# illini-robomaster/irmv_detection

Hardware: AMD Instinct MI355X
Metric: end-to-end FPS (preprocess→NMS→PnP) 640×640 YOLOv8n, 1/2/4/8 MI355X (higher is better)
Workload: dtype f16

## Files before the change

### irmv_detection_amd/csrc/engine.cpp

```cpp
#include "engine_internal.hpp"

static thread_local std::string g_err;
int irmv::fail(int code, const std::string &msg) { g_err = msg; return code; }

extern "C" const char *irmv_last_error(void) { return g_err.c_str(); }
extern "C" const char *irmv_version(void)
{
    static char buf[96];
    static std::once_flag once;
    std::call_once(once, [] {
        int v = 0;
        if (hipRuntimeGetVersion(&v) != hipSuccess) v = 0;
        snprintf(buf, sizeof buf, "irmv_hip 0.3 (gfx950; HIP runtime %d)", v);
    });
    return buf;
}
extern "C" int irmv_device_synchronize(int device)
{
    HIP_TRY(hipSetDevice(device));
    HIP_TRY(hipDeviceSynchronize());
    return IRMV_OK;
}
extern "C" int irmv_device_count(int *count)
{
// ... 188 lines not shown
    cfg->armor_min_large_center_distance = 3.2; cfg->armor_max_large_center_distance = 5.5;
    cfg->src_format = IRMV_SRC_HWC8;
    cfg->bayer_gain_q8[0] = cfg->bayer_gain_q8[1] = cfg->bayer_gain_q8[2] = 256;
}

static EngineSwitches read_switches()
{
    auto set = [](const char *name) { return getenv(name) != nullptr; };
    auto starts = [](const char *name, char c) { const char *v = getenv(name); return v && v[0] == c; };
    auto off = [&](const char *name) { return starts(name, '0'); };
    auto is1 = [&](const char *name) { return starts(name, '1'); };
    EngineSwitches s;
    TuneSwitches &t = s.tune;
    t.untuned = off("IRMV_AUTOTUNE"); t.verbose = set("IRMV_AUTOTUNE_VERBOSE"); t.warn = set("IRMV_TUNE_WARN");
    const char *s2 = getenv("IRMV_FORCE_S2"), *wres = getenv("IRMV_FORCE_WRES");
    t.has_s2 = s2 != nullptr; t.force_s2 = s2 ? s2 : "";
    t.has_wres = wres != nullptr; t.force_wres = wres ? wres : "";
    t.force_pw = set("IRMV_FORCE_PW"); t.force_pwn = set("IRMV_FORCE_PWN"); t.force_cm = set("IRMV_FORCE_CM");
    t.force_w8 = set("IRMV_FORCE_W8"); t.force_nt8 = set("IRMV_FORCE_NT8"); t.force_pf4 = set("IRMV_FORCE_PF4");
    t.no_pw = set("IRMV_NO_PW"); t.no_pwn = set("IRMV_NO_PWN"); t.no_pf2 = set("IRMV_NO_PF2"); t.no_pf4 = set("IRMV_NO_PF4");
    t.no_cm = set("IRMV_NO_CM"); t.no_w8 = set("IRMV_NO_W8"); t.no_nt8 = set("IRMV_NO_NT8"); t.no_wres = set("IRMV_NO_WRES");
    t.no_deep = is1("IRMV_NO_DEEP");
    s.front.fastx = !off("IRMV_FRONT_FASTX"); s.front.direct = !off("IRMV_FRONT_DIRECT"); s.front.tall = !off("IRMV_FRONT_TILE8");
    s.fused_front = !off("IRMV_FUSED_FRONT"); s.fused_c2f = !off("IRMV_FUSED_C2F"); s.bneck64 = !off("IRMV_BNECK64"); s.kpt3 = !off("IRMV_KPT3");
    s.fused_head = !off("IRMV_FUSED_HEAD");
    s.merge_head0 = off("IRMV_MERGE_HEAD0") ? 0 : (is1("IRMV_MERGE_HEAD0") ? 1 : -1);
    s.group_head = !off("IRMV_GROUP_HEAD"); s.group_verbose = set("IRMV_GROUP_VERBOSE"); s.group_force = set("IRMV_GROUP_FORCE");
    if (const char *ns = getenv("IRMV_STREAMS")) { s.has_streams = true; s.streams = atoi(ns); }
    s.numa = !off("IRMV_NUMA");
    s.inline_copies = is1("IRMV_INLINE_COPIES"); s.graph_upload = !off("IRMV_GRAPH_UPLOAD"); s.window_upload = !off("IRMV_WINDOW_UPLOAD");
    if (const char *uk = getenv("IRMV_UPLOAD_KERNEL")) s.upload_kernel_blocks = atoi(uk);
    s.sync_launch = starts("IRMV_SYNC_LAUNCH", 'e') ? 1 : (starts("IRMV_SYNC_LAUNCH", 'g') ? 0 : -1);
    s.split_scan = !off("IRMV_SPLIT_SCAN"); s.emit_scan = !off("IRMV_EMIT_SCAN");
    s.sparse_head = !off("IRMV_SPARSE_HEAD"); s.sparse_branch = !off("IRMV_SPARSE_BRANCH");
    s.zero_copy_results = !off("IRMV_ZERO_COPY_RESULTS"); s.post_keys_only = is1("IRMV_POST_KEYS_ONLY");
    s.nms_classwalk = !off("IRMV_NMS_CLASSWALK");
    s.nms_prefilter = off("IRMV_NMS_PREFILTER") ? 0 : 1;
    if (const char *pe = getenv("IRMV_NMS_PRE")) { int hi = 0, lo = 0; if (sscanf(pe, "%d,%d", &hi, &lo) == 2 && hi >= 64 && hi <= 512 && lo >= 32 && lo < hi) s.nms_prefilter = hi | (lo << 16); }
    if (const char *st = getenv("IRMV_NMS_STAMPS")) { s.nms_stamps = true; s.nms_stamps_slots = atoi(st); }
    return s;
}

constexpr size_t kCfgSizeV1 = offsetof(irmv_engine_cfg, src_format);
constexpr size_t kCfgSizeV2 = offsetof(irmv_engine_cfg, reserved2);
static_assert(offsetof(irmv_engine_cfg, net_height) < kCfgSizeV2 && kCfgSizeV2 < sizeof(irmv_engine_cfg), "three distinct cfg sizes");
static_assert(offsetof(irmv_engine_cfg, win_width) == offsetof(irmv_engine_cfg, reserved2) + 4 && offsetof(irmv_engine_cfg, win_height) + 2 == sizeof(irmv_engine_cfg),
              "win_width / win_height fill the tail of irmv_engine_cfg");

static irmv_engine_cfg window_view(const irmv_engine_cfg &c)
{
    irmv_engine_cfg v = c;
    if (c.win_width > 0 && c.win_height > 0) { v.src_width = c.win_width; v.src_height = c.win_height; }
    v.win_width = v.win_height = 0;
    return v;
}

static int resolve_cfg(const irmv_engine_cfg *cfg_in, irmv_engine_cfg *full)
{
    const size_t sz = cfg_in->struct_size;
    if (sz != sizeof(irmv_engine_cfg) && sz != kCfgSizeV1 && sz != kCfgSizeV2) return fail(IRMV_ERR_ARG, "irmv_engine_cfg size mismatch");
    if (sz != sizeof(irmv_engine_cfg)) {
        irmv_engine_cfg_default(full);
        memcpy(full, cfg_in, sz == kCfgSizeV1 ? kCfgSizeV1 : offsetof(irmv_engine_cfg, net_height));
        full->struct_size = sizeof *full;
        full->bayer_demosaic = IRMV_DEMOSAIC_BILINEAR;
    } else {
        *full = *cfg_in;
// ... 339 lines not shown
```

### irmv_detection_amd/csrc/engine_internal.hpp

```cpp
#pragma once
#include <hip/hip_runtime.h>

#include <algorithm>
#include <chrono>
#include <cmath>
#include <cstdio>
#include <cstring>
#include <fstream>
#include <map>
#include <mutex>
#include <set>
#include <memory>
#include <string>
#include <vector>

#include "../../include/irmv_hip.h"
#include "irmv_common.hpp"
#include "numa.hpp"

using namespace irmv;

namespace irmv { int fail(int code, const std::string &msg); }
#define HIP_TRY(expr)                                                                                 \
    do {                                                                                              \
// ... 27 lines not shown
};

struct SegRef { int t = -1, coff = 0, C = 0, shift = 0; };

struct FrontSwitches { bool fastx = true, direct = true, tall = true; };

struct TuneSwitches {
    bool untuned, verbose, warn;
    bool has_s2, has_wres;
    std::string force_s2, force_wres;
    bool force_pw, force_pwn, force_cm, force_w8, force_nt8, force_pf4;
    bool no_pw, no_pwn, no_pf2, no_pf4, no_cm, no_w8, no_nt8, no_wres, no_deep;
};

struct EngineSwitches {
    TuneSwitches tune{};
    FrontSwitches front;
    bool fused_front = true, fused_c2f = true;
    bool bneck64 = true;
    bool kpt3 = true;
    bool fused_head = true;
    int merge_head0 = -1;
    bool group_head = true;
    bool group_verbose = false;
    bool group_force = false;
    bool has_streams = false; int streams = 0;
    bool numa = true;
    bool inline_copies = false;
    bool graph_upload = true;
    int upload_kernel_blocks = 256;
    bool window_upload = true;
    int sync_launch = -1;
    bool split_scan = true;
    bool emit_scan = true, sparse_head = true, sparse_branch = true;
    bool zero_copy_results = true;
    bool post_keys_only = false;
    bool nms_classwalk = true;
    int nms_prefilter = 1;
    bool nms_stamps = false; int nms_stamps_slots = 0;
};

enum OpKind { OP_PRE, OP_CONV0, OP_CONV, OP_POOL, OP_NMS, OP_LIGHT, OP_FRONT, OP_C2F2, OP_C2F32, OP_DW, OP_SHUF, OP_SCAN, OP_BNECK, OP_KPT3, OP_DEMOSAIC, OP_CROP };

struct Op {
    OpKind kind;
    std::string layer;
    ConvCfg cfg{};
    ConvCfg cfg_one{};
    char kname_one[48] = {0};
    SegRef s0, s1;
    int Hin = 0, Win = 0, Hout = 0, Wout = 0, cin = 0, cout = 0, cout_pad = 0, ksteps = 0;
    int out_t = -1, out_coff = 0, res_t = -1, res_coff = 0;
    half_t *w_packed = nullptr;
    half_t *w_k16 = nullptr;
    half_t *w_lds[4] = {nullptr, nullptr, nullptr, nullptr};
    float *bias = nullptr;
    double flops = 0, bytes = 0;
    double w_bytes = 0;
    double out_bytes = 0;
    bool pair = false;
    int level = -1;
    char kname[48] = {0};
    int sub[4] = {-1, -1, -1, -1};
    int mode = 0;
    bool shortcut = false;
    int fuse_next = -1;
// ... 167 lines not shown
```

### irmv_detection_amd/csrc/engine_plan.cpp

```cpp
#include "engine_internal.hpp"

static bool is_cls_final_carrier(const Op &op) { return op.fuse_next >= 0 && op.level >= 0 && op.layer.rfind("model.22.cv3.", 0) == 0; }

void irmv::finalize_head_fusion(irmv_engine *e)
{
    for (Op &op : e->ops) {
        if (op.fuse_next < 0) continue;
        const bool k16 = op.cfg.cin16 && !op.cfg.lds && !op.cfg_one.lds && !op.cfg.deep && !op.cfg_one.deep && op.cfg.nt == 1 && op.cfg_one.nt == 1 && e->ops[op.fuse_next].w_k16;
        const bool ok = k16 || (op.cfg.lds && op.cfg.nt == 4 && op.cfg_one.lds && op.cfg_one.nt == 4);
        if (!ok) { op.fuse_next = -1; continue; }
        e->ops[op.fuse_next].fused_away = true;
        e->lazy_tensors.insert(e->tensors[op.out_t].name);
        const size_t l = strlen(op.kname), l1 = strlen(op.kname_one);
        snprintf(op.kname + l, sizeof op.kname - l, "+1x1");
        snprintf(op.kname_one + l1, sizeof op.kname_one - l1, "+1x1");
    }
    int fused = 0;
    for (const Op &op : e->ops) fused += is_cls_final_carrier(op);
    e->emit_scan = e->sw.split_scan && fused == 3 && e->sw.emit_scan;
    e->sparse_head = e->emit_scan && e->cand_bits && e->sw.sparse_head;
    e->sparse_branch = e->sparse_head && e->sw.sparse_branch;
}

static bool is_box_final_carrier(const Op &op) { return op.fuse_next >= 0 && op.level >= 0 && op.layer.rfind("model.22.cv2.", 0) == 0; }

static void sparse_head_plan(irmv_engine *e, std::vector<Launch> &plan)
{
    int last_cls = -1;
    bool lvl_cls[3] = {false, false, false};
    for (size_t i = 0; i < plan.size(); i++)
        if (plan[i].scan && plan[i].group < 0) { last_cls = (int)i; lvl_cls[e->ops[plan[i].op].level] = true; }
    auto box_carrier = [&](const Launch &l) {
        const Op &op = e->ops[l.op];
        return l.group < 0 && l.fused && op.kind == OP_CONV && is_box_final_carrier(op) && op.level < 3 && lvl_cls[op.level];
    };
    std::vector<char> first_conv(plan.size(), 0);
    if (e->sparse_branch)
        for (size_t i = 0; i < plan.size(); i++) {
            const Launch &f = plan[i];
            const Op &fo = e->ops[f.op];
            if (f.group >= 0 || f.fused || f.scan || fo.kind != OP_CONV || !(f.cfg_one ? fo.cfg_one : fo.cfg).wr || fo.res_t >= 0) continue;
            int carrier = -1;
            for (size_t j = i + 1; j < plan.size(); j++) {
                const Op &co = e->ops[plan[j].op];
                if (box_carrier(plan[j]) && co.level == fo.level && co.s0.t == fo.out_t && co.s1.C == 0 && co.s0.coff == fo.out_coff && co.Hin == fo.Hout && co.Win == fo.Wout) carrier = plan[j].op;
            }
            bool other = false;
            for (int k = 0; k < (int)e->ops.size(); k++) {
                const Op &o = e->ops[k];
                if (k == carrier || k == f.op) continue;
                other = other || o.s0.t == fo.out_t || o.s1.t == fo.out_t || o.res_t == fo.out_t || o.out_t == fo.out_t;
            }
            first_conv[i] = carrier >= 0 && !other;
        }
    std::vector<Launch> out, moved;
    for (size_t i = 0; i < plan.size(); i++) {
        Launch &l = plan[i];
        Op &op = e->ops[l.op];
        if (l.scan) {
            if (l.group < 0) l.bytes -= e->ops[op.fuse_next].out_bytes;
            else for (size_t m = 0; m < e->head_groups[l.group].members.size(); m++)
                if (l.scan >> m & 1u) l.bytes -= e->ops[e->ops[e->head_groups[l.group].members[m]].fuse_next].out_bytes;
        }
        const bool cls_first = op.level >= 0 && op.level < 3 && lvl_cls[op.level];
        const bool box = box_carrier(l);
        const bool kpt = op.kind == OP_KPT3 && cls_first && (int)i > last_cls;
        if (box || kpt) {
            l.sparse = true;
            l.bytes -= box ? e->ops[op.fuse_next].out_bytes : op.out_bytes;
            if (e->sparse_branch) l.gate = 1;
        }
        if (first_conv[i]) {
            l.gate = 2;
            op.gated_first = true;
// ... 54 lines not shown
```

### irmv_detection_amd/csrc/irmv_common.hpp

```cpp
#pragma once

#include <hip/hip_runtime.h>

#include <cstdint>
#include <cstdlib>

namespace irmv {

typedef _Float16 half_t;
typedef _Float16 half8 __attribute__((ext_vector_type(8)));
typedef _Float16 half4 __attribute__((ext_vector_type(4)));
typedef float f32x4 __attribute__((ext_vector_type(4)));

constexpr float kActScale = 1.44269504088896341f;
constexpr float kActUnscale = 0.693147180559945309f;
typedef unsigned int u32x4_t __attribute__((ext_vector_type(4)));
__device__ __forceinline__ float silu_rcp(float y) { return __builtin_amdgcn_rcpf(1.0f + __builtin_amdgcn_exp2f(-y)); }
__device__ __forceinline__ unsigned int silu_pack2(float y0, float y1)
{
    const float r0 = silu_rcp(y0), r1 = silu_rcp(y1);
    unsigned int o;
    asm("v_fma_mixlo_f16 %0, %1, %2, 0" : "=v"(o) : "v"(y0), "v"(r0));
    asm("v_fma_mixhi_f16 %0, %1, %2, 0" : "+v"(o) : "v"(y1), "v"(r1));
    return o;
// ... 245 lines not shown
    const half_t *wl;
    int tiles_x, tiles_y, twc_log2, patch_bytes, batch, tile2d;
    int gx, gy;
};
struct LdsMultiArgs {
    int n;
    int start[kMultiMax + 1];
    LdsMember m[kMultiMax];
};
struct DirectMultiArgs {
    int n;
    int start[kMultiMax + 1], gx[kMultiMax], gy[kMultiMax];
    ConvArgs a[kMultiMax];
};

struct ConvCfg {
    int ks, stride, mt, nt; bool cin16; int act; bool out_f32; bool lds; int ipw;
    bool deep;
    bool ct;
    bool pw;
    bool pf2;
    bool pf4;
    bool w8;
    int cm;
    bool wr;
    bool pp;
};
struct ConvWeights { const half_t *w_packed; const half_t *w_lds[4]; const half_t *w_k16; };
struct ConvLaunch;
bool resolve_conv(const ConvCfg &cfg, const ConvArgs &a, const ConvWeights &w, int batch, ConvLaunch *out = nullptr);
bool launch_conv(const ConvCfg &cfg, const ConvArgs &a, const ConvWeights &w, int batch, hipStream_t s);
const char *conv_cfg_name(const ConvCfg &cfg, char *buf, int n);
bool conv_pw_eligible(const ConvCfg &cfg, const ConvArgs &a);
bool conv_lds_fits(const ConvArgs &a, const ConvWeights &w, int stride, int mt, int nt);
int conv_wres_tiles(const ConvArgs &a, int stride, bool pp);
bool launch_conv_lds_multi(int nt, const ConvArgs *a, const ConvWeights *w, int n, int batch, hipStream_t s);
bool launch_conv_direct_multi(const ConvCfg &cfg, const ConvArgs *a, int n, hipStream_t s);

void launch_sppf_pool(half_t *buf, int batch, int H, int W, int C, hipStream_t s);
int sppf_slab(int batch, int H, int W, int C);

struct DevDet {
    float box_net[4];
    float xyxy[4];
    float score;
    int32_t cls, anchor, pnp_ok;
    float kpts_net[8];
    float kpts[8];
    double rvec[3], tvec[3], quat[4];
    int32_t armor_valid;
    int32_t armor_size;
    int32_t n_lights;
    int32_t pad_;
};
struct DevFrameOut { int32_t num_dets, n_candidates, overflow, pad; };

struct PnpConst {
    double fx, fy, cx, cy, k1, k2, p1, p2, k3;
    double hy[2], hz[2];
};

struct PostArgs {
    const float *head_all;
    int slots_total, first;
    float *boxes;
    unsigned long long *keys;
// ... 78 lines not shown
```

### irmv_detection_amd/csrc/k_conv.hip

```cpp
#include "irmv_common.hpp"

#include <algorithm>
#include <cstdio>
#include <cstring>
#include <iterator>
#include <mutex>
#include <type_traits>

namespace irmv {

template <int MT, int NT>
struct PrefetchDepth { static constexpr int value = (MT * NT >= 8) ? 2 : ((MT * NT >= 4) ? 3 : 4); };
template <int MT, int NT>
struct DeepPrefetchDepth { static constexpr int value = (MT + NT <= 2) ? 12 : ((MT + NT <= 3) ? 10 : 6); };


template <int KS, int STRIDE, int MT, int NT, bool CIN16, int ACT, bool OUT_F32, bool CT = false, bool DEEP = false>
__device__ __forceinline__ void conv_mfma_body(const ConvArgs &a, int wg_x, int wg_y, int grid_x, int grid_y)
{
    constexpr int PAD = KS / 2;
    constexpr int PF = DEEP ? DeepPrefetchDepth<MT, NT>::value : PrefetchDepth<MT, NT>::value;
    static_assert(!CT || (KS == 3 && !CIN16), "chunk-major order is the 3x3 LDS family's");
    const int lane = threadIdx.x & 63, wave = threadIdx.x >> 6;
    const int g = lane >> 4, r = lane & 15;
// ... 605 lines not shown
    const int units = (a.M + 15) / 16;
    int wg = (cus[dev] * per_cu[dev] + groups - 1) / groups;
    if (wg > (units + 7) / 8) wg = (units + 7) / 8;
    if (wg < 1) wg = 1;
    hipLaunchKernelGGL((conv1x1_pwn_kernel<KS, NBW>), dim3(wg, groups), dim3(512), lds, s, a, wg);
}

static constexpr struct { int ksteps, nbw; ConvLauncher launch; } k_pw[] = {
    {4, 1, launch_pw_inst<4>}, {6, 1, launch_pw_inst<6>}, {8, 1, launch_pw_inst<8>}, {12, 1, launch_pw_inst<12>}, {16, 1, launch_pw_inst<16>},
    {4, 2, launch_pwn_inst<4, 2>}, {6, 2, launch_pwn_inst<6, 2>}, {8, 2, launch_pwn_inst<8, 2>}, {12, 2, launch_pwn_inst<12, 2>}, {16, 2, launch_pwn_inst<16, 2>},
    {4, 4, launch_pwn_inst<4, 4>}, {6, 4, launch_pwn_inst<6, 4>}, {8, 4, launch_pwn_inst<8, 4>},
};

static ConvLauncher pick_pw(const ConvCfg &c, const ConvArgs &a, LdsGeom &g)
{
    const int nbw = c.ipw > 1 ? c.ipw : 1;
    if (!conv_pw_eligible(c, a) || a.cout_pad % (64 * nbw) != 0) return nullptr;
    for (const auto &v : k_pw)
        if (v.ksteps == a.ksteps && v.nbw == nbw) {
            g.bytes = (size_t)nbw * 4 * a.ksteps * 1024 + (nbw > 1 ? (size_t)nbw * 64 * 4 : 0);
            return v.launch;
        }
    return nullptr;
}

constexpr int lds_pmax(int stride, int mt, bool tile2d, int wr = 0, int pf = 0)
{
    return pf == 2 ? (stride == 1 ? 4 : 8) : (wr ? 4 : ((tile2d && stride == 1) ? (mt == 4 ? 8 : 4) : 12));
}

#ifndef IRMV_LDS_WAVES
#define IRMV_LDS_WAVES 2
#endif
template <int STRIDE, int MT, int NT, bool TILE2D, int N2, int PF = 0, int CM = 0, int NWV = 4, int WR = 0, bool PP = false>
__device__ __forceinline__ void conv3x3_lds_body(const ConvArgs &a, const half_t *wl, int tiles_x, int tiles_y, int twc_log2, int a_patch_bytes, int ipw, int batch,
                                                 int wg_x, int wg_y, int grid_x, int grid_y, int stagger = 0)
{
    extern __shared__ __attribute__((aligned(16))) unsigned char smem[];
    const int lane = threadIdx.x & 63, wave = threadIdx.x >> 6, tid = threadIdx.x;
    constexpr bool PF2 = PF != 0;
    constexpr int NPF = PF == 2 ? 4 : (PF == 1 ? 2 : 1);
    constexpr int NTH = 64 * NWV;
    static_assert(!PP || (WR > 0 && NWV % 2 == 0), "ping-pong groups share resident weights");
    constexpr int NWP = PP ? NWV / 2 : NWV;
    constexpr int NTP = 64 * NWP;
    const int sub = PP ? wave / NWP : 0, wv = wave - sub * NWP, tidp = tid - sub * NTP;
    const int g = lane >> 4, r = lane & 15;
    const int bx = wg_x, by = wg_y;
    (void)grid_x; (void)grid_y;
    const int wg_tiles = PP ? (tiles_x * tiles_y + 1) / 2 : tiles_x * tiles_y;
    const int grp = bx / wg_tiles;
    int tile = PP ? 2 * (bx - grp * wg_tiles) + sub : bx - grp * wg_tiles;
    const bool active = tile < tiles_x * tiles_y;
    if (!active) tile = 0;
    const int img = grp * ipw, nimg = min(ipw, batch - img);
    const int nblk = by;
    const int HWo = a.Hout * a.Wout;
    bool gated = false;
    unsigned int l_mask = 0u;
    int l_pos = 0;
    int n_mine = nimg, n_max = nimg;
    if constexpr (WR > 0) {
        auto gate_images = [&](int t) -> unsigned int {
            const int h = a.tile_gate - 1;
            int nseg, lo0, len, pitch;
            if constexpr (TILE2D) {
                const int TWc = 1 << twc_log2, RH = NWP * MT * (16 >> twc_log2);
                const int tyi = t / tiles_x, txi = t - tyi * tiles_x;
                const int ya = max(tyi * RH - h, 0), yb = min(tyi * RH + RH + h, a.Hout);
                const int xa = max(txi * TWc - h, 0), xb = min(txi * TWc + TWc + h, a.Wout);
                nseg = yb - ya; lo0 = ya * a.Wout + xa; len = xb - xa; pitch = a.Wout;
            } else {
                constexpr int TPX = 16 * NWP * MT;
                const int lo = max(t * TPX - h * (a.Wout + 1), 0), hi = min(min(t * TPX + TPX, HWo) + h * (a.Wout + 1), HWo);
                nseg = 1; lo0 = lo; len = hi - lo; pitch = 0;
            }
            const int wps = (len + 62) >> 5, items = nseg * wps;
            unsigned int m = 0u;
            for (int j0 = 0; j0 < items; j0 += 64) {
                const int it = j0 + lane, sg = it / wps, bl = a.scan_abase + lo0 + sg * pitch, wd = (bl >> 5) + (it - sg * wps);
                const int s0 = max(bl - wd * 32, 0), s1 = min(bl + len - wd * 32, 32);
                const bool item = it < items && s1 > s0;
                const unsigned int bm = item ? (0xffffffffu >> (32 - (s1 - s0))) << s0 : 0u;
                for (int i0 = 0; i0 < nimg; i0 += 16) {
                    unsigned int cw[16];
#pragma unroll
                    for (int i = 0; i < 16; i++) cw[i] = i0 + i < nimg ? a.cand_bits[(unsigned int)((img + i0 + i) * a.cand_words + (item ? wd : 0))] : 0u;
#pragma unroll
                    for (int i = 0; i < 16; i++) m |= __ballot((cw[i] & bm) != 0u) != 0ull ? 1u << ((i0 + i) & 31) : 0u;
                }
            }
            return (unsigned int)__builtin_amdgcn_readfirstlane((int)m);
        };
        gated = a.tile_gate != 0 && a.cand_bits != nullptr && nimg <= 32;
        if (gated) {
// ... 64 lines not shown
    constexpr int PMAX = lds_pmax(STRIDE, MT, TILE2D, WR, PF);
    constexpr int WPT = (9 * NT * 64 + NTH - 1) / NTH;
    const int n_pe = PR * PW * 4;
    const float inv_pw = 1.0f / (float)PW;
    const half_t *src_p[PMAX];
    int dst_p[PMAX];
    bool val_p[PMAX], use_p[PMAX];
#pragma unroll
    for (int i = 0; i < PMAX; i++) {
        const int e = tidp + i * NTP;
        use_p[i] = e < n_pe;
        val_p[i] = false;
        src_p[i] = a.s0.p;
        dst_p[i] = 0;
        if (i * NTP >= n_pe) continue;
        const int pix = use_p[i] ? (e >> 2) : 0, q = e & 3;
        int pr = (int)((float)pix * inv_pw);
        pr -= (pr * PW > pix) ? 1 : 0;
        pr += ((pr + 1) * PW <= pix) ? 1 : 0;
        const int pc = pix - pr * PW;
        const int iy = iy_base + pr, ix = ix_base + pc;
        val_p[i] = active && use_p[i] && (unsigned)iy < (unsigned)a.Hin && (unsigned)ix < (unsigned)a.Win;
        src_p[i] = a.s0.p + ((size_t)(img * a.Hin + (val_p[i] ? iy : 0)) * a.Win + (val_p[i] ? ix : 0)) * a.s0.ld + q * 8;
        dst_p[i] = pix * pix_stride(STRIDE) + q * 16;
    }
    const half8 *wsrc = reinterpret_cast<const half8 *>(wl) + (size_t)nblk * chunks * (9 * NT * 64);

    const half8 *w2 = s_w2 + lane;

    half8 rp[NPF][PMAX], rw[NPF][WPT];
    const size_t img_stride = (size_t)a.Hin * a.Win * a.s0.ld;
    int l_im = 0, l_chunk = 0;
    int c_im = 0, c_chunk = 0;
    auto issue_loads = [&](half8 (&p)[PMAX], half8 (&w)[WPT]) {
        const size_t off = (size_t)l_im * img_stride + (size_t)l_chunk * 32;
#pragma unroll
        for (int i = 0; i < PMAX; i++) {
            p[i] = zero8;
            if (val_p[i]) p[i] = *reinterpret_cast<const half8 *>(src_p[i] + off);
        }
#pragma unroll
        for (int i = 0; i < WPT; i++) {
            if (CM > 0 && l_im != 0) break;
            const int e = tid + i * NTH;
            if (e < 9 * NT * 64) w[i] = wsrc[(size_t)l_chunk * (9 * NT * 64) + e];
        }
        if constexpr (CM > 0) {
            if (++l_im == nimg) { l_im = 0; l_chunk++; }
        } else {
            if (++l_chunk == chunks) { l_chunk = 0; l_im++; }
        }
    };
    auto write_lds = [&](const half8 (&p)[PMAX], const half8 (&w)[WPT]) {
#pragma unroll
        for (int i = 0; i < PMAX; i++) {
            if (use_p[i]) *reinterpret_cast<half8 *>(s_patch + dst_p[i]) = p[i];
        }
#pragma unroll
        for (int i = 0; i < WPT; i++) {
            if (CM > 0 && c_im != 0) break;
            const int e = tid + i * NTH;
            if (e < 9 * NT * 64) s_w[e] = w[i];
        }
    };

    constexpr int NA = CM > 0 ? CM : 1;
    f32x4 acc[NA][MT][NT];
#pragma unroll
    for (int nt = 0; nt < NT; nt++) {
        const int ch = (NT % 2 == 0) ? (by * NT * 16 + (nt >> 1) * 32 + g * 8 + (nt & 1) * 4) : (a.pair ? ((by >> 1) * 32 + g * 8 + (by & 1) * 4) : (by * 16 + g * 4));
        const f32x4 b0 = *reinterpret_cast<const f32x4 *>(a.bias + ch);
#pragma unroll
        for (int ai = 0; ai < NA; ai++)
#pragma unroll
            for (int mt = 0; mt < MT; mt++) acc[ai][mt][nt] = b0;
    }

    const int nt0 = nblk * NT;
    auto store_tile = [&](int im, auto ai_) {
        auto &accx = acc[decltype(ai_)::value];
        half8 W2[N2 > 0 ? N2 : 1][2];
        if constexpr (N2 > 0) {
#pragma unroll
// ... 82 lines not shown
                                            const int idx = atomicAdd(&a.scan_counts[im], 1);
                                            const unsigned int u = __float_as_uint(v2[i]);
                                            const unsigned int ord = (u & 0x80000000u) ? ~u : (u | 0x80000000u);
                                            if (idx >= 0 && idx < a.scan_key_cap)
                                                a.scan_keys[(size_t)im * a.scan_key_cap + idx] =
                                                    ((unsigned long long)ord << 32) | (unsigned long long)(0xffffffffu - (unsigned int)(an * a.scan_nc + co + i));
                                        }
                                    }
                                }
                            }
                        }
                    }
                } else {
                    const int t = nt0;
                    const int c0 = a.pair ? ((t >> 1) * 32 + g * 8 + (t & 1) * 4) : (t * 16 + g * 4);
                    half4 o;
                    if (a.res) {
#pragma unroll
                        for (int i = 0; i < 4; i++) o[i] = silu_add_res(accx[mt][0][i], (float)rv4[mt][i]);
                    } else {
                        o = silu_pack4(accx[mt][0][0], accx[mt][0][1], accx[mt][0][2], accx[mt][0][3]);
                    }
                    *reinterpret_cast<half4 *>(static_cast<half_t *>(a.out) + m * a.out_ld + c0) = o;
                }
            }
#pragma unroll
            for (int nt = 0; nt < NT; nt++)
                accx[mt][nt] = (NT % 2 == 0) ? (f32x4){bs[nt >> 1][(nt & 1) * 4 + 0], bs[nt >> 1][(nt & 1) * 4 + 1], bs[nt >> 1][(nt & 1) * 4 + 2], bs[nt >> 1][(nt & 1) * 4 + 3]}
                                             : (f32x4){bs[0][0], bs[0][1], bs[0][2], bs[0][3]};
        }
    };

    using I0 = std::integral_constant<int, 0>;
    const int steps = nimg * chunks;
    constexpr int NPIECE = PMAX + WPT, PER_TAP = (NPIECE + 8) / 9;
    auto taps = [&](auto spread, auto ai_, int plane = 0) {
        constexpr bool SPREAD = decltype(spread)::value;
        auto &accx = acc[decltype(ai_)::value];
        const unsigned char *s_pl = s_patch + (size_t)plane * a_patch_bytes;
        const half8 *s_wc = s_w + plane * (9 * NT * 64);
        size_t off = 0;
        if constexpr (SPREAD) {
            if (l_im == nimg) { l_im = nimg - 1; l_chunk = chunks - 1; }
            off = (size_t)l_im * img_stride + (size_t)l_chunk * 32;
        }
#pragma unroll
        for (int tap = 0; tap < 9; tap++) {
            if constexpr (SPREAD) {
#pragma unroll
                for (int k = 0; k < PER_TAP; k++) {
                    const int j = tap * PER_TAP + k;
                    if (j < PMAX) {
                        rp[0][j] = zero8;
                        if (val_p[j]) rp[0][j] = *reinterpret_cast<const half8 *>(src_p[j] + off);
                    } else if (j < NPIECE) {
                        const int e = tid + (j - PMAX) * NTH;
                        if (e < 9 * NT * 64) rw[0][j - PMAX] = wsrc[(size_t)l_chunk * (9 * NT * 64) + e];
                    }
                }
            }
            const int kh = tap / 3, kw = tap - kh * 3;
            const int toff = (kh * PW + kw) * pix_stride(STRIDE);
            half8 A[NT], B[MT];
#pragma unroll
            for (int nt = 0; nt < NT; nt++) A[nt] = s_wc[(tap * NT + nt) * 64 + lane];
#pragma unroll
            for (int mt = 0; mt < MT; mt++) B[mt] = *reinterpret_cast<const half8 *>(s_pl + poff[mt] + toff);
#pragma unroll
            for (int mt = 0; mt < MT; mt++)
#pragma unroll
                for (int nt = 0; nt < NT; nt++)
                    accx[mt][nt] = __builtin_amdgcn_mfma_f32_16x16x32_f16(A[nt], B[mt], accx[mt][nt], 0, 0, 0);
            if constexpr (SPREAD) __builtin_amdgcn_sched_barrier(0x38f);
        }
        if constexpr (SPREAD) {
            if (++l_chunk == chunks) { l_chunk = 0; l_im++; }
        }
    };
    auto ksteps_wr = [&]() {
        constexpr int KS = (WR > 0 ? WR : 1) * 9;
        auto &accx = acc[0];
        half8 A[2][NT], B[2][MT];
        auto frag = [&](auto ks_, half8 (&Af)[NT], half8 (&Bf)[MT]) {
            constexpr int ks = decltype(ks_)::value, c = ks / 9, tap = ks % 9, kh = tap / 3, kw = tap % 3;
            const unsigned char *s_pl = s_patch + (size_t)c * a_patch_bytes + (kh * PW + kw) * pix_stride(STRIDE);
            const half8 *s_wc = s_w + (c * 9 + tap) * (NT * 64) + lane;
#pragma unroll
            for (int nt = 0; nt < NT; nt++) Af[nt] = s_wc[nt * 64];
#pragma unroll
            for (int mt = 0; mt < MT; mt++) Bf[mt] = *reinterpret_cast<const half8 *>(s_pl + poff[mt]);
        };
        frag(std::integral_constant<int, 0>{}, A[0], B[0]);
        auto step = [&](auto ks_) {
            constexpr int ks = decltype(ks_)::value;
            if constexpr (ks + 1 < KS) frag(std::integral_constant<int, ks + 1>{}, A[(ks + 1) & 1], B[(ks + 1) & 1]);
            __builtin_amdgcn_sched_barrier(0);
#pragma unroll
            for (int mt = 0; mt < MT; mt++)
#pragma unroll
                for (int nt = 0; nt < NT; nt++)
                    accx[mt][nt] = __builtin_amdgcn_mfma_f32_16x16x32_f16(A[ks & 1][nt], B[ks & 1][mt], accx[mt][nt], 0, 0, 0);
            __builtin_amdgcn_sched_barrier(0);
        };
        auto run = [&](auto self, auto ks_) -> void {
            constexpr int ks = decltype(ks_)::value;
            if constexpr (ks < KS) { step(ks_); self(self, std::integral_constant<int, ks + 1>{}); }
        };
        run(run, std::integral_constant<int, 0>{});
    };
// ... 94 lines not shown
            if constexpr (CM > 2) f(std::integral_constant<int, 2>{});
            if constexpr (CM > 3) f(std::integral_constant<int, 3>{});
        };
        issue_loads(rp[0], rw[0]);
        for (int c = 0; c < chunks; c++) {
            each_image([&](auto ai) {
                constexpr int AI = decltype(ai)::value;
                if (AI < nimg) {
                    write_lds(rp[0], rw[0]);
                    __syncthreads();
                    if (!(c == chunks - 1 && AI == nimg - 1)) issue_loads(rp[0], rw[0]);
                    taps(std::false_type{}, ai);
                    __syncthreads();
                    if (++c_im == nimg) { c_im = 0; c_chunk++; }
                }
            });
        }
        each_image([&](auto ai) {
            if (decltype(ai)::value < nimg) store_tile(img + decltype(ai)::value, ai);
        });
    } else if constexpr (!PF2) {
        issue_loads(rp[0], rw[0]);
        for (int s = 0; s < steps; s++) {
            write_lds(rp[0], rw[0]);
            __syncthreads();
            if constexpr (MT == 4) {
                taps(std::true_type{}, I0{});
            } else {
                if (s + 1 < steps) issue_loads(rp[0], rw[0]);
                taps(std::false_type{}, I0{});
            }
            __syncthreads();
            if (++c_chunk == chunks) {
                store_tile(img + c_im, I0{});
                c_chunk = 0;
                c_im++;
            }
        }
    } else {
#pragma unroll
        for (int k = 0; k < NPF; k++)
            if (k < steps) issue_loads(rp[k], rw[k]);
        for (int s = 0; s < steps; s += NPF) {
#pragma unroll
            for (int k = 0; k < NPF; k++) {
                if (s + k < steps) {
                    write_lds(rp[k], rw[k]);
                    __syncthreads();
                    if (s + k + NPF < steps) issue_loads(rp[k], rw[k]);
                    mma_step();
                }
            }
        }
    }
}

template <int STRIDE, int MT, int NT, bool TILE2D, int N2, int PF = 0, int CM = 0, int NWV = 4, int WR = 0, bool PP = false>
__global__ __launch_bounds__(64 * NWV) __attribute__((amdgpu_waves_per_eu(IRMV_LDS_WAVES))) void conv3x3_lds_kernel(ConvArgs a, const half_t *wl, int tiles_x, int tiles_y, int twc_log2, int a_patch_bytes, int ipw, int batch, int nblocks, int xcd)
{
    const int wg_tiles = PP ? (tiles_x * tiles_y + 1) / 2 : tiles_x * tiles_y, groups = (batch + ipw - 1) / ipw;
    int rem, grp;
    tile_image(blockIdx.x, wg_tiles * nblocks, groups, xcd & 1, rem, grp);
    const int nblk = rem / wg_tiles, tile = rem - nblk * wg_tiles;
    conv3x3_lds_body<STRIDE, MT, NT, TILE2D, N2, PF, CM, NWV, WR, PP>(a, wl, tiles_x, tiles_y, twc_log2, a_patch_bytes, ipw, batch, grp * wg_tiles + tile, nblk, wg_tiles * groups, nblocks, (xcd >> 1) & 1);
}

template <int STRIDE, int MT, int NT>
__global__ __launch_bounds__(256) __attribute__((amdgpu_waves_per_eu(IRMV_LDS_WAVES))) void conv3x3_lds_multi(LdsMultiArgs m)
{
    int id = blockIdx.x, k = 0;
    while (k + 1 < m.n && id >= m.start[k + 1]) k++;
    id -= m.start[k];
    const LdsMember &l = m.m[k];
    const int wx = id % l.gx, wy = id / l.gx;
#define IRMV_BODY(T2D_, N2_) conv3x3_lds_body<STRIDE, MT, NT, T2D_, N2_>(l.a, l.wl, l.tiles_x, l.tiles_y, l.twc_log2, l.patch_bytes, 1, l.batch, wx, wy, l.gx, l.gy)
    if constexpr (NT == 4) {
        if (l.a.n2 == 4) { if (l.tile2d) IRMV_BODY(true, 4); else IRMV_BODY(false, 4); return; }
        if (l.a.n2 == 1) { if (l.tile2d) IRMV_BODY(true, 1); else IRMV_BODY(false, 1); return; }
    }
    if (l.tile2d) IRMV_BODY(true, 0); else IRMV_BODY(false, 0);
#undef IRMV_BODY
}

static LdsGeom lds_geom(const ConvArgs &a, int stride, int mt, int nt, int nwv = 4, int wr = 0, bool pp = false, int pf = 0)
{
    LdsGeom g{false, 0, 0, 0, 0, 0};
    if (a.Cin % 32 != 0 || a.s1.C != 0 || a.s0.shift != 0) return g;
    if (!((nt == 1) || ((nt == 2 || nt == 4) && a.pair) || (nt == 8 && a.pair && nwv == 8 && stride == 2 && mt == 1))) return g;
    if (a.cout_pad % (16 * nt) != 0) return g;
    int pr, pw;
    const int l2 = a.Wout % 16 == 0 ? 4 : (a.Wout % 8 == 0 ? 3 : (a.Wout % 4 == 0 ? 2 : -1));
    const int rh = l2 >= 0 ? nwv * mt * (16 >> l2) : 0;
    if (l2 >= 0 && a.Hout % rh == 0) {
        g.tile2d = true;
        g.twc_log2 = l2;
        g.tiles_x = a.Wout >> l2;
        g.tiles_y = a.Hout / rh;
        pr = rh * stride + 2;
        pw = (1 << l2) * stride + 2;
    } else {
        const int tpx = 16 * nwv * mt;
        g.tiles_x = (a.Hout * a.Wout + tpx - 1) / tpx;
        g.tiles_y = 1;
        const int rows = (tpx + a.Wout - 2) / a.Wout + 1;
        pr = (rows - 1) * stride + 3;
        pw = a.Win + 2;
    }
    if ((size_t)pr * pw * 4 > (size_t)lds_pmax(stride, mt, g.tile2d, wr, pf) * 64 * nwv) return g;
    g.patch_bytes = pr * pw * pix_stride(stride);
    const int planes = wr ? wr : 1;
    const size_t bytes = (size_t)planes * (pp ? 2 : 1) * g.patch_bytes + (size_t)planes * 9 * nt * 1024 + 512 + (size_t)a.n2 * 2048;
    if (bytes > (size_t)(wr ? 160 : (nwv == 8 ? 150 : 80)) * 1024) return g;
    g.bytes = bytes;
    return g;
}

static const half_t *lds_weights(const ConvWeights &w, int nt) { return w.w_lds[nt == 8 ? 3 : (nt == 4 ? 2 : (nt == 2 ? 1 : 0))]; }

bool conv_lds_fits(const ConvArgs &a, const ConvWeights &w, int stride, int mt, int nt)
{
    return lds_weights(w, nt) && lds_geom(a, stride, mt, nt).bytes > 0;
}

template <int STRIDE, int MT, int NT, bool TILE2D, int N2, int PF = 0, int CM = 0, int NWV = 4, int WR = 0, bool PP = false>
static void launch_lds_inst(const ConvLaunch &l, hipStream_t s)
{
    static unsigned long long attr_done = 0;
    once_per_device(attr_done, [] {
        (void)hipFuncSetAttribute(reinterpret_cast<const void *>(conv3x3_lds_kernel<STRIDE, MT, NT, TILE2D, N2, PF, CM, NWV, WR, PP>), hipFuncAttributeMaxDynamicSharedMemorySize, 160 * 1024);
    });
    const LdsGeom &g = l.g;
    const int groups = (l.batch + l.ipw - 1) / l.ipw;
    const int wg_tiles = PP ? (g.tiles_x * g.tiles_y + 1) / 2 : g.tiles_x * g.tiles_y;
    const int nblocks = l.a.cout_pad / (16 * NT);
    hipLaunchKernelGGL((conv3x3_lds_kernel<STRIDE, MT, NT, TILE2D, N2, PF, CM, NWV, WR, PP>), dim3(wg_tiles * groups * nblocks), dim3(64 * NWV), g.bytes, s, l.a,
                       l.w, g.tiles_x, g.tiles_y, g.twc_log2, g.patch_bytes, l.ipw, l.batch, nblocks, xcd_image_order() | (wres_stagger() << 1));
}

static LdsGeom wres_geom(const ConvArgs &a, int stride, bool pp)
{
    if (stride != 1 || a.Cin != 64 || a.cout_pad != 64 || !a.pair || (a.n2 > 0 && a.res) || !(a.n2 == 0 || a.n2 == 1 || a.n2 == 4)) return LdsGeom{false, 0, 0, 0, 0, 0};
    LdsGeom g = pp ? lds_geom(a, 1, 2, 4, 4, 2, true) : lds_geom(a, 1, 2, 4, 8, 2);
    if (pp && !g.tile2d) g.bytes = 0;
    return g;
}
int conv_wres_tiles(const ConvArgs &a, int stride, bool pp)
{
    const LdsGeom g = wres_geom(a, stride, pp);
    if (!g.bytes) return 0;
    return pp ? (g.tiles_x * g.tiles_y + 1) / 2 : g.tiles_x * g.tiles_y;
}

struct LdsKey { int stride, mt, nt, n2, pf, cm, nwv, wr, pp; };
struct LdsVariant { LdsKey key; ConvLauncher launch[2]; };

template <int ST, int MT, int NT, int N2 = 0, int PF = 0, int CM = 0, int NWV = 4, int WR = 0, bool PP = false>
constexpr LdsVariant lds_variant()
{
    LdsVariant v{{ST, MT, NT, N2, PF, CM, NWV, WR, PP}, {nullptr, launch_lds_inst<ST, MT, NT, true, N2, PF, CM, NWV, WR, PP>}};
    if constexpr (!PP) v.launch[0] = launch_lds_inst<ST, MT, NT, false, N2, PF, CM, NWV, WR, PP>;
    return v;
}

static constexpr LdsVariant k_lds[] = {
    lds_variant<1, 1, 1>(), lds_variant<1, 2, 1>(), lds_variant<1, 4, 1>(),
    lds_variant<1, 1, 2>(), lds_variant<1, 2, 2>(), lds_variant<1, 4, 2>(),
    lds_variant<1, 1, 4>(), lds_variant<1, 2, 4>(), lds_variant<1, 4, 4>(),
    lds_variant<2, 1, 1>(), lds_variant<2, 2, 1>(), lds_variant<2, 4, 1>(),
    lds_variant<2, 1, 2>(), lds_variant<2, 2, 2>(), lds_variant<2, 4, 2>(),
    lds_variant<2, 1, 4>(), lds_variant<2, 2, 4>(), lds_variant<2, 4, 4>(),
    lds_variant<1, 1, 4, 1>(), lds_variant<1, 2, 4, 1>(), lds_variant<1, 4, 4, 1>(),
    lds_variant<1, 1, 4, 4>(), lds_variant<1, 2, 4, 4>(), lds_variant<1, 4, 4, 4>(),
    lds_variant<1, 1, 1, 0, 1>(), lds_variant<1, 1, 2, 0, 1>(), lds_variant<1, 1, 4, 0, 1>(),
    lds_variant<2, 1, 1, 0, 1>(), lds_variant<2, 1, 2, 0, 1>(), lds_variant<2, 1, 4, 0, 1>(),
    lds_variant<1, 1, 1, 0, 2>(), lds_variant<2, 1, 1, 0, 2>(),
    lds_variant<1, 1, 4, 0, 0, 4>(), lds_variant<1, 1, 4, 0, 0, 2>(), lds_variant<1, 2, 4, 0, 0, 2>(),
    lds_variant<2, 1, 4, 0, 0, 4>(), lds_variant<2, 1, 4, 0, 0, 2>(), lds_variant<2, 2, 4, 0, 0, 2>(),
    lds_variant<1, 1, 4, 1, 0, 4>(), lds_variant<1, 2, 4, 1, 0, 2>(), lds_variant<1, 1, 4, 4, 0, 4>(), lds_variant<1, 2, 4, 4, 0, 2>(),
    lds_variant<2, 2, 4, 0, 0, 0, 8>(), lds_variant<2, 2, 4, 0, 0, 2, 8>(), lds_variant<2, 1, 4, 0, 0, 0, 8>(), lds_variant<2, 1, 4, 0, 0, 4, 8>(),
    lds_variant<2, 1, 8, 0, 0, 0, 8>(), lds_variant<2, 1, 8, 0, 0, 2, 8>(),
    lds_variant<1, 2, 4, 0, 0, 0, 8, 2>(), lds_variant<1, 2, 4, 1, 0, 0, 8, 2>(), lds_variant<1, 2, 4, 4, 0, 0, 8, 2>(),
    lds_variant<1, 2, 4, 0, 0, 0, 8, 2, true>(), lds_variant<1, 2, 4, 1, 0, 0, 8, 2, true>(), lds_variant<1, 2, 4, 4, 0, 0, 8, 2, true>(),
};

static ConvLauncher pick_lds(const ConvCfg &c, const ConvArgs &a, int ipw, LdsGeom &g)
{
    const int pf = c.pf4 ? 2 : (c.pf2 ? 1 : 0), nwv = c.w8 || c.wr ? 8 : 4;
    if (c.cm && c.cm != ipw) return nullptr;
    if (a.n2 > 0 && (a.cout_pad != 64 || !a.pair || a.res)) return nullptr;
    g = c.wr ? wres_geom(a, c.stride, c.pp) : lds_geom(a, c.stride, c.mt, c.nt, nwv, 0, false, pf);
    if (!g.bytes) return nullptr;
    const LdsKey key{c.stride, c.mt, c.nt, a.n2, pf, c.cm, nwv, c.wr ? 2 : 0, c.pp};
    for (const LdsVariant &v : k_lds)
        if (!memcmp(&v.key, &key, sizeof key)) return v.launch[g.tile2d];
    return nullptr;
}

static ConvLauncher pick_direct(const ConvCfg &c)
{
    const int mi = c.mt == 1 ? 0 : (c.mt == 2 ? 1 : 2), ni = c.nt == 1 ? 0 : (c.nt == 2 ? 1 : 2);
    if (c.mt != 1 << mi || c.nt != 1 << ni) return nullptr;
    const DirectKey key{c.ks, c.stride, c.cin16, c.act, c.out_f32, c.ct, c.deep};
    for (const DirectVariant &v : k_direct)
        if (!memcmp(&v.key, &key, sizeof key)) return v.tile[mi][ni];
    return nullptr;
}

bool resolve_conv(const ConvCfg &c, const ConvArgs &a, const ConvWeights &w, int batch, ConvLaunch *out)
{
    if (a.cout_pad % (16 * c.nt) != 0) return false;
    ConvLaunch local;
    ConvLaunch &l = out ? *out : local;
    l.launch = nullptr; l.a = a; l.w = w.w_packed; l.batch = batch; l.ipw = c.ipw < 1 ? 1 : c.ipw; l.g = LdsGeom{false, 0, 0, 0, 0, 0};
    if (w.w_k16) {
        if (a.Cin == 16 && a.cout_pad == 16 && a.s1.C == 0 && a.s0.shift == 0) l.launch = launch_k16;
        l.w = l.a.w2 = w.w_k16;
    } else if (c.pw) {
        l.launch = pick_pw(c, a, l.g);
    } else if (c.lds) {
        l.w = lds_weights(w, c.nt);
        if (l.w) l.launch = pick_lds(c, a, l.ipw, l.g);
    } else if (!c.wr) {
        if (c.ct) l.w = a.n2 > 0 ? nullptr : w.w_lds[0];
        if (l.w) l.launch = pick_direct(c);
        l.a.w = l.w;
// ... 208 lines not shown
```

Before: 65080.

## Extend sparse tile gating to non-resident LDS 3x3 convs in the head

Adds a gated (GT) variant of the LDS 3x3 conv kernel that walks only the images whose candidate mask marks the tile as live, skipping loads, MMA steps and stores for the rest. The sparse-head planner now also treats plain stride-1 LDS convs as eligible for gating (behind a default-on switch), not only weight-resident ones. This avoids computing head convolutions on regions with no detection candidates, at the cost of extra template instantiations and per-image mask bookkeeping in the load and store loops.

```diff
diff --git a/irmv_detection_amd/csrc/engine.cpp b/irmv_detection_amd/csrc/engine.cpp
--- a/irmv_detection_amd/csrc/engine.cpp
+++ b/irmv_detection_amd/csrc/engine.cpp
@@ -244,7 +244,7 @@
     if (const char *uk = getenv("IRMV_UPLOAD_KERNEL")) s.upload_kernel_blocks = atoi(uk);
     s.sync_launch = starts("IRMV_SYNC_LAUNCH", 'e') ? 1 : (starts("IRMV_SYNC_LAUNCH", 'g') ? 0 : -1);
     s.split_scan = !off("IRMV_SPLIT_SCAN"); s.emit_scan = !off("IRMV_EMIT_SCAN");
-    s.sparse_head = !off("IRMV_SPARSE_HEAD"); s.sparse_branch = !off("IRMV_SPARSE_BRANCH");
+    s.sparse_head = !off("IRMV_SPARSE_HEAD"); s.sparse_branch = !off("IRMV_SPARSE_BRANCH"); s.sparse_first = !off("IRMV_SPARSE_FIRST");
     s.zero_copy_results = !off("IRMV_ZERO_COPY_RESULTS"); s.post_keys_only = is1("IRMV_POST_KEYS_ONLY");
     s.nms_classwalk = !off("IRMV_NMS_CLASSWALK");
     s.nms_prefilter = off("IRMV_NMS_PREFILTER") ? 0 : 1;
diff --git a/irmv_detection_amd/csrc/engine_internal.hpp b/irmv_detection_amd/csrc/engine_internal.hpp
--- a/irmv_detection_amd/csrc/engine_internal.hpp
+++ b/irmv_detection_amd/csrc/engine_internal.hpp
@@ -83,6 +83,7 @@
     bool window_upload = true;
     int sync_launch = -1;
     bool split_scan = true;
+    bool sparse_first = true;
     bool emit_scan = true, sparse_head = true, sparse_branch = true;
     bool zero_copy_results = true;
     bool post_keys_only = false;
diff --git a/irmv_detection_amd/csrc/engine_plan.cpp b/irmv_detection_amd/csrc/engine_plan.cpp
--- a/irmv_detection_amd/csrc/engine_plan.cpp
+++ b/irmv_detection_amd/csrc/engine_plan.cpp
@@ -39,7 +39,8 @@
         for (size_t i = 0; i < plan.size(); i++) {
             const Launch &f = plan[i];
             const Op &fo = e->ops[f.op];
-            if (f.group >= 0 || f.fused || f.scan || fo.kind != OP_CONV || !(f.cfg_one ? fo.cfg_one : fo.cfg).wr || fo.res_t >= 0) continue;
+            const ConvCfg &fc = f.cfg_one ? fo.cfg_one : fo.cfg;
+            if (f.group >= 0 || f.fused || f.scan || fo.kind != OP_CONV || !(e->sw.sparse_first ? conv_cfg_gates(fc) : fc.wr) || fo.res_t >= 0) continue;
             int carrier = -1;
             for (size_t j = i + 1; j < plan.size(); j++) {
                 const Op &co = e->ops[plan[j].op];
diff --git a/irmv_detection_amd/csrc/irmv_common.hpp b/irmv_detection_amd/csrc/irmv_common.hpp
--- a/irmv_detection_amd/csrc/irmv_common.hpp
+++ b/irmv_detection_amd/csrc/irmv_common.hpp
@@ -301,6 +301,7 @@
 bool launch_conv(const ConvCfg &cfg, const ConvArgs &a, const ConvWeights &w, int batch, hipStream_t s);
 const char *conv_cfg_name(const ConvCfg &cfg, char *buf, int n);
 bool conv_pw_eligible(const ConvCfg &cfg, const ConvArgs &a);
+bool conv_cfg_gates(const ConvCfg &cfg);
 bool conv_lds_fits(const ConvArgs &a, const ConvWeights &w, int stride, int mt, int nt);
 int conv_wres_tiles(const ConvArgs &a, int stride, bool pp);
 bool launch_conv_lds_multi(int nt, const ConvArgs *a, const ConvWeights *w, int n, int batch, hipStream_t s);
diff --git a/irmv_detection_amd/csrc/k_conv.hip b/irmv_detection_amd/csrc/k_conv.hip
--- a/irmv_detection_amd/csrc/k_conv.hip
+++ b/irmv_detection_amd/csrc/k_conv.hip
@@ -661,7 +661,7 @@
 #ifndef IRMV_LDS_WAVES
 #define IRMV_LDS_WAVES 2
 #endif
-template <int STRIDE, int MT, int NT, bool TILE2D, int N2, int PF = 0, int CM = 0, int NWV = 4, int WR = 0, bool PP = false>
+template <int STRIDE, int MT, int NT, bool TILE2D, int N2, int PF = 0, int CM = 0, int NWV = 4, int WR = 0, bool PP = false, bool GT = false>
 __device__ __forceinline__ void conv3x3_lds_body(const ConvArgs &a, const half_t *wl, int tiles_x, int tiles_y, int twc_log2, int a_patch_bytes, int ipw, int batch,
                                                  int wg_x, int wg_y, int grid_x, int grid_y, int stagger = 0)
 {
@@ -671,6 +671,7 @@
     constexpr int NPF = PF == 2 ? 4 : (PF == 1 ? 2 : 1);
     constexpr int NTH = 64 * NWV;
     static_assert(!PP || (WR > 0 && NWV % 2 == 0), "ping-pong groups share resident weights");
+    static_assert(!GT || (WR == 0 && CM == 0 && PF == 0 && N2 == 0 && NWV == 4), "gated chunked form: image-major, one step of lead, plain epilogue");
     constexpr int NWP = PP ? NWV / 2 : NWV;
     constexpr int NTP = 64 * NWP;
     const int sub = PP ? wave / NWP : 0, wv = wave - sub * NWP, tidp = tid - sub * NTP;
@@ -689,7 +690,7 @@
     unsigned int l_mask = 0u;
     int l_pos = 0;
     int n_mine = nimg, n_max = nimg;
-    if constexpr (WR > 0) {
+    if constexpr (WR > 0 || GT) {
         auto gate_images = [&](int t) -> unsigned int {
             const int h = a.tile_gate - 1;
             int nseg, lo0, len, pitch;
@@ -820,8 +821,17 @@
     const size_t img_stride = (size_t)a.Hin * a.Win * a.s0.ld;
     int l_im = 0, l_chunk = 0;
     int c_im = 0, c_chunk = 0;
+    unsigned int c_mask = l_mask;
+    int l_img = 0, c_img = 0;
+    auto listed = [&](unsigned int &mask, int pos) {
+        if (!gated) return pos;
+        const int i = __builtin_ctz(mask);
+        mask &= mask - 1u;
+        return i;
+    };
+    if constexpr (GT) { l_img = listed(l_mask, 0); c_img = listed(c_mask, 0); }
     auto issue_loads = [&](half8 (&p)[PMAX], half8 (&w)[WPT]) {
-        const size_t off = (size_t)l_im * img_stride + (size_t)l_chunk * 32;
+        const size_t off = (size_t)(GT ? l_img : l_im) * img_stride + (size_t)l_chunk * 32;
 #pragma unroll
         for (int i = 0; i < PMAX; i++) {
             p[i] = zero8;
@@ -836,7 +846,10 @@
         if constexpr (CM > 0) {
             if (++l_im == nimg) { l_im = 0; l_chunk++; }
         } else {
-            if (++l_chunk == chunks) { l_chunk = 0; l_im++; }
+            if (++l_chunk == chunks) {
+                l_chunk = 0; l_im++;
+                if constexpr (GT) { if (l_im < n_mine) l_img = listed(l_mask, l_im); }
+            }
         }
     };
     auto write_lds = [&](const half8 (&p)[PMAX], const half8 (&w)[WPT]) {
@@ -985,7 +998,7 @@
     };
 
     using I0 = std::integral_constant<int, 0>;
-    const int steps = nimg * chunks;
+    const int steps = (GT ? n_mine : nimg) * chunks;
     constexpr int NPIECE = PMAX + WPT, PER_TAP = (NPIECE + 8) / 9;
     auto taps = [&](auto spread, auto ai_, int plane = 0) {
         constexpr bool SPREAD = decltype(spread)::value;
@@ -994,8 +1007,12 @@
         const half8 *s_wc = s_w + plane * (9 * NT * 64);
         size_t off = 0;
         if constexpr (SPREAD) {
-            if (l_im == nimg) { l_im = nimg - 1; l_chunk = chunks - 1; }
-            off = (size_t)l_im * img_stride + (size_t)l_chunk * 32;
+            if constexpr (GT) {
+                if (l_im == n_mine) { l_im = n_mine - 1; l_chunk = chunks - 1; }
+            } else {
+                if (l_im == nimg) { l_im = nimg - 1; l_chunk = chunks - 1; }
+            }
+            off = (size_t)(GT ? l_img : l_im) * img_stride + (size_t)l_chunk * 32;
         }
 #pragma unroll
         for (int tap = 0; tap < 9; tap++) {
@@ -1027,7 +1044,10 @@
             if constexpr (SPREAD) __builtin_amdgcn_sched_barrier(0x38f);
         }
         if constexpr (SPREAD) {
-            if (++l_chunk == chunks) { l_chunk = 0; l_im++; }
+            if (++l_chunk == chunks) {
+                l_chunk = 0; l_im++;
+                if constexpr (GT) { if (l_im < n_mine) l_img = listed(l_mask, l_im); }
+            }
         }
     };
     auto ksteps_wr = [&]() {
@@ -1188,9 +1208,10 @@
             }
             __syncthreads();
             if (++c_chunk == chunks) {
-                store_tile(img + c_im, I0{});
+                store_tile(img + (GT ? c_img : c_im), I0{});
                 c_chunk = 0;
                 c_im++;
+                if constexpr (GT) { if (c_im < n_mine) c_img = listed(c_mask, c_im); }
             }
         }
     } else {
@@ -1211,14 +1232,14 @@
     }
 }
 
-template <int STRIDE, int MT, int NT, bool TILE2D, int N2, int PF = 0, int CM = 0, int NWV = 4, int WR = 0, bool PP = false>
+template <int STRIDE, int MT, int NT, bool TILE2D, int N2, int PF = 0, int CM = 0, int NWV = 4, int WR = 0, bool PP = false, bool GT = false>
 __global__ __launch_bounds__(64 * NWV) __attribute__((amdgpu_waves_per_eu(IRMV_LDS_WAVES))) void conv3x3_lds_kernel(ConvArgs a, const half_t *wl, int tiles_x, int tiles_y, int twc_log2, int a_patch_bytes, int ipw, int batch, int nblocks, int xcd)
 {
     const int wg_tiles = PP ? (tiles_x * tiles_y + 1) / 2 : tiles_x * tiles_y, groups = (batch + ipw - 1) / ipw;
     int rem, grp;
     tile_image(blockIdx.x, wg_tiles * nblocks, groups, xcd & 1, rem, grp);
     const int nblk = rem / wg_tiles, tile = rem - nblk * wg_tiles;
-    conv3x3_lds_body<STRIDE, MT, NT, TILE2D, N2, PF, CM, NWV, WR, PP>(a, wl, tiles_x, tiles_y, twc_log2, a_patch_bytes, ipw, batch, grp * wg_tiles + tile, nblk, wg_tiles * groups, nblocks, (xcd >> 1) & 1);
+    conv3x3_lds_body<STRIDE, MT, NT, TILE2D, N2, PF, CM, NWV, WR, PP, GT>(a, wl, tiles_x, tiles_y, twc_log2, a_patch_bytes, ipw, batch, grp * wg_tiles + tile, nblk, wg_tiles * groups, nblocks, (xcd >> 1) & 1);
 }
 
 template <int STRIDE, int MT, int NT>
@@ -1278,18 +1299,18 @@
     return lds_weights(w, nt) && lds_geom(a, stride, mt, nt).bytes > 0;
 }
 
-template <int STRIDE, int MT, int NT, bool TILE2D, int N2, int PF = 0, int CM = 0, int NWV = 4, int WR = 0, bool PP = false>
+template <int STRIDE, int MT, int NT, bool TILE2D, int N2, int PF = 0, int CM = 0, int NWV = 4, int WR = 0, bool PP = false, bool GT = false>
 static void launch_lds_inst(const ConvLaunch &l, hipStream_t s)
 {
     static unsigned long long attr_done = 0;
     once_per_device(attr_done, [] {
-        (void)hipFuncSetAttribute(reinterpret_cast<const void *>(conv3x3_lds_kernel<STRIDE, MT, NT, TILE2D, N2, PF, CM, NWV, WR, PP>), hipFuncAttributeMaxDynamicSharedMemorySize, 160 * 1024);
+        (void)hipFuncSetAttribute(reinterpret_cast<const void *>(conv3x3_lds_kernel<STRIDE, MT, NT, TILE2D, N2, PF, CM, NWV, WR, PP, GT>), hipFuncAttributeMaxDynamicSharedMemorySize, 160 * 1024);
     });
     const LdsGeom &g = l.g;
     const int groups = (l.batch + l.ipw - 1) / l.ipw;
     const int wg_tiles = PP ? (g.tiles_x * g.tiles_y + 1) / 2 : g.tiles_x * g.tiles_y;
     const int nblocks = l.a.cout_pad / (16 * NT);
-    hipLaunchKernelGGL((conv3x3_lds_kernel<STRIDE, MT, NT, TILE2D, N2, PF, CM, NWV, WR, PP>), dim3(wg_tiles * groups * nblocks), dim3(64 * NWV), g.bytes, s, l.a,
+    hipLaunchKernelGGL((conv3x3_lds_kernel<STRIDE, MT, NT, TILE2D, N2, PF, CM, NWV, WR, PP, GT>), dim3(wg_tiles * groups * nblocks), dim3(64 * NWV), g.bytes, s, l.a,
                        l.w, g.tiles_x, g.tiles_y, g.twc_log2, g.patch_bytes, l.ipw, l.batch, nblocks, xcd_image_order() | (wres_stagger() << 1));
 }
 
@@ -1307,15 +1328,22 @@
     return pp ? (g.tiles_x * g.tiles_y + 1) / 2 : g.tiles_x * g.tiles_y;
 }
 
-struct LdsKey { int stride, mt, nt, n2, pf, cm, nwv, wr, pp; };
+struct LdsKey { int stride, mt, nt, n2, pf, cm, nwv, wr, pp, gt; };
 struct LdsVariant { LdsKey key; ConvLauncher launch[2]; };
 
-template <int ST, int MT, int NT, int N2 = 0, int PF = 0, int CM = 0, int NWV = 4, int WR = 0, bool PP = false>
+template <int ST, int MT, int NT, int N2 = 0, int PF = 0, int CM = 0, int NWV = 4, int WR = 0, bool PP = false, bool GT = false>
 constexpr LdsVariant lds_variant()
 {
-    LdsVariant v{{ST, MT, NT, N2, PF, CM, NWV, WR, PP}, {nullptr, launch_lds_inst<ST, MT, NT, true, N2, PF, CM, NWV, WR, PP>}};
-    if constexpr (!PP) v.launch[0] = launch_lds_inst<ST, MT, NT, false, N2, PF, CM, NWV, WR, PP>;
+    LdsVariant v{{ST, MT, NT, N2, PF, CM, NWV, WR, PP, GT}, {nullptr, launch_lds_inst<ST, MT, NT, true, N2, PF, CM, NWV, WR, PP, GT>}};
+    if constexpr (!PP) v.launch[0] = launch_lds_inst<ST, MT, NT, false, N2, PF, CM, NWV, WR, PP, GT>;
     return v;
+}
+template <int MT, int NT> constexpr LdsVariant lds_gated() { return lds_variant<1, MT, NT, 0, 0, 0, 4, 0, false, true>(); }
+
+bool conv_cfg_gates(const ConvCfg &c)
+{
+    if (c.pw || (!c.lds && !c.wr)) return false;
+    return c.wr || (c.stride == 1 && !c.pf2 && !c.pf4 && !c.w8 && c.cm == 0);
 }
 
 static constexpr LdsVariant k_lds[] = {
@@ -1337,6 +1365,9 @@
     lds_variant<2, 1, 8, 0, 0, 0, 8>(), lds_variant<2, 1, 8, 0, 0, 2, 8>(),
     lds_variant<1, 2, 4, 0, 0, 0, 8, 2>(), lds_variant<1, 2, 4, 1, 0, 0, 8, 2>(), lds_variant<1, 2, 4, 4, 0, 0, 8, 2>(),
     lds_variant<1, 2, 4, 0, 0, 0, 8, 2, true>(), lds_variant<1, 2, 4, 1, 0, 0, 8, 2, true>(), lds_variant<1, 2, 4, 4, 0, 0, 8, 2, true>(),
+    lds_gated<1, 1>(), lds_gated<2, 1>(), lds_gated<4, 1>(),
+    lds_gated<1, 2>(), lds_gated<2, 2>(), lds_gated<4, 2>(),
+    lds_gated<1, 4>(), lds_gated<2, 4>(), lds_gated<4, 4>(),
 };
 
 static ConvLauncher pick_lds(const ConvCfg &c, const ConvArgs &a, int ipw, LdsGeom &g)
@@ -1346,7 +1377,8 @@
     if (a.n2 > 0 && (a.cout_pad != 64 || !a.pair || a.res)) return nullptr;
     g = c.wr ? wres_geom(a, c.stride, c.pp) : lds_geom(a, c.stride, c.mt, c.nt, nwv, 0, false, pf);
     if (!g.bytes) return nullptr;
-    const LdsKey key{c.stride, c.mt, c.nt, a.n2, pf, c.cm, nwv, c.wr ? 2 : 0, c.pp};
+    const int gt = !c.wr && a.n2 == 0 && a.tile_gate != 0 && a.cand_bits != nullptr && conv_cfg_gates(c);
+    const LdsKey key{c.stride, c.mt, c.nt, a.n2, pf, c.cm, nwv, c.wr ? 2 : 0, c.pp, gt};
     for (const LdsVariant &v : k_lds)
         if (!memcmp(&v.key, &key, sizeof key)) return v.launch[g.tile2d];
     return nullptr;
```

Result: no change. 65000 (median of 2 runs) (-0.1%).
